# khanhptnk/psketch

Hardware: NVIDIA B200
Metric: env-steps/s (step+features+expert) (higher is better)
Workload: dtype u8

## Files before the change

### psketch_b200/csrc/psk_craft.cu

```cuda
#include <cstdio>
#include <cstdlib>
#include <cstring>
#include <atomic>
#include <mutex>

#include "psk_common.cuh"

namespace psk {

template <int W, int H, class TAB>
__device__ __forceinline__ void step_env(const TAB &st, Agent &a, uint8_t *row,
                                         const uint8_t *rd, int act, uint32_t &flags) {
    int x = a.x(), y = a.y(), dir = a.dir();
    if (act < 4) {
        dir = act;
        const int tx = x + dx_of(act), ty = y + dy_of(act);
        if (tx >= 0 && ty >= 0 && tx < W && ty < H && rd[tx * H + ty] == 0) {
            x = tx;
            y = ty;
        }
        a.set_pose(x, y, dir);
    } else if (act == PSK_ACT_USE) {
        const int fx = x + dx_of(dir), fy = y + dy_of(dir);
        if (fx >= 0 && fy >= 0 && fx < W && fy < H) {
// ... 1091 lines not shown
    const uint32_t buf_s = wbuf_s + (USE_TMA ? (uint32_t)(it & 1) * feature_tile_bytes(true, EPW, nf, 4) : 0u);
    const uint32_t trash_s = buf_s + feature_tile_bytes(USE_TMA, EPW, nf, VEC_ESZ) - 16;
    const int n16 = EPW * nf / 4;
    if (USE_TMA) {
        if (lane == 0) bulk_wait_read<1>();
        __syncwarp();
        if (KC > 0) {
#pragma unroll
            for (int i = 0; i < (n16 + 31) / 32; i++)
                if (i * 32 + lane < n16) sts_zero16(buf_s + (i * 32 + lane) * 16);
        } else {
            for (int i = lane; i < n16; i += 32) sts_zero16(buf_s + i * 16);
        }
        __syncwarp();
    }
    if (le < ne)
        scatter_features<W, H, WIN, TPE, ESZ>(buf_s + le * nf * ESZ, trash_s, cells, a, K, j);
    const uint32_t bytes = (uint32_t)ne * (uint32_t)nf * 4u;
    const bool vec_ok = (bytes & 15u) == 0 && (reinterpret_cast<uintptr_t>(gdst) & 15) == 0;
    if (USE_TMA) {
        if (vec_ok) {
            fence_async_smem();
            __syncwarp();
            if (lane == 0) bulk_store(gdst, buf_s, bytes);
        } else {
            __syncwarp();
            for (int i = lane; i < ne * nf; i += 32) {
                float t;
                asm volatile("ld.shared.f32 %0, [%1];" : "=f"(t) : "r"(buf_s + i * 4));
                gdst[i] = t;
            }
            __syncwarp();
        }
    } else if (ESZ == 4) {
        __syncwarp();
        if (vec_ok) {
            float4 *g4 = reinterpret_cast<float4 *>(gdst);
            const int m16 = (int)(bytes / 16);
            auto move16 = [&](int i) {
                float4 t;
                asm volatile("ld.shared.v4.f32 {%0,%1,%2,%3}, [%4];"
                             : "=f"(t.x), "=f"(t.y), "=f"(t.z), "=f"(t.w)
                             : "r"(buf_s + i * 16));
                sts_zero16(buf_s + i * 16);
                store_out16(g4 + i, t);
            };
            if (KC > 0 && m16 == n16) {
                constexpr int NIT = (EPW * (2 * WIN * WIN * KC + KC + 5) / 4 + 31) / 32;
#pragma unroll
                for (int i0 = 0; i0 < NIT; i0 += 4) {
                    float4 t[4];
#pragma unroll
                    for (int u = 0; u < 4; u++) {
                        const int i = (i0 + u) * 32 + lane;
                        if (i0 + u < NIT && i < n16)
                            asm volatile("ld.shared.v4.f32 {%0,%1,%2,%3}, [%4];"
                                         : "=f"(t[u].x), "=f"(t[u].y), "=f"(t[u].z), "=f"(t[u].w)
                                         : "r"(buf_s + i * 16));
                    }
#pragma unroll
                    for (int u = 0; u < 4; u++) {
                        const int i = (i0 + u) * 32 + lane;
                        if (i0 + u < NIT && i < n16) sts_zero16(buf_s + i * 16);
                    }
#pragma unroll
                    for (int u = 0; u < 4; u++) {
                        const int i = (i0 + u) * 32 + lane;
                        if (i0 + u < NIT && i < n16) store_out16(g4 + i, t[u]);
                    }
                }
            } else {
                for (int i = lane; i < m16; i += 32) move16(i);
                for (int i = m16 + lane; i < n16; i += 32) sts_zero16(buf_s + i * 16);
            }
        } else {
            for (int i = lane; i < ne * nf; i += 32) {
                float t;
                asm volatile("ld.shared.f32 %0, [%1];" : "=f"(t) : "r"(buf_s + i * 4));
                gdst[i] = t;
            }
            __syncwarp();
            for (int i = lane; i < n16; i += 32) sts_zero16(buf_s + i * 16);
        }
        __syncwarp();
    } else {
        __syncwarp();
        if (vec_ok) {
            float4 *g4 = reinterpret_cast<float4 *>(gdst);
            const int m16 = (int)(bytes / 16);
            auto move16 = [&](int i) {
                uint32_t w;
                asm volatile("ld.shared.u32 %0, [%1];" : "=r"(w) : "r"(buf_s + i * 4));
                asm volatile("st.shared.u32 [%0], %1;" ::"r"(buf_s + i * 4), "r"(0) : "memory");
                store_out16(g4 + i, widen_u8x4(w));
            };
            if (KC > 0 && m16 == n16) {
                constexpr int NIT = (EPW * (2 * WIN * WIN * KC + KC + 5) / 4 + 31) / 32;
#pragma unroll
                for (int i0 = 0; i0 < NIT; i0 += 4) {
                    uint32_t w[4];
#pragma unroll
                    for (int u = 0; u < 4; u++) {
                        const int i = (i0 + u) * 32 + lane;
                        if (i0 + u < NIT && i < n16)
                            asm volatile("ld.shared.u32 %0, [%1];" : "=r"(w[u]) : "r"(buf_s + i * 4));
                    }
#pragma unroll
                    for (int u = 0; u < 4; u++) {
                        const int i = (i0 + u) * 32 + lane;
                        if (i0 + u < NIT && i < n16)
                            asm volatile("st.shared.u32 [%0], %1;" ::"r"(buf_s + i * 4), "r"(0) : "memory");
                    }
#pragma unroll
                    for (int u = 0; u < 4; u++) {
                        const int i = (i0 + u) * 32 + lane;
                        if (i0 + u < NIT && i < n16) store_out16(g4 + i, widen_u8x4(w[u]));
                    }
                }
            } else {
                for (int i = lane; i < m16; i += 32) move16(i);
                for (int i = m16 + lane; i < n16; i += 32)
                    asm volatile("st.shared.u32 [%0], %1;" ::"r"(buf_s + i * 4), "r"(0) : "memory");
            }
        } else {
            for (int i = lane; i < ne * nf; i += 32) {
                uint32_t b;
                asm volatile("ld.shared.u8 %0, [%1];" : "=r"(b) : "r"(buf_s + i));
                gdst[i] = (float)b;
            }
            __syncwarp();
            for (int i = lane; i < n16; i += 32)
                asm volatile("st.shared.u32 [%0], %1;" ::"r"(buf_s + i * 4), "r"(0) : "memory");
        }
        __syncwarp();
    }
}

template <int W, int H, int WIN, int TPE, int KC>
__device__ __forceinline__ void warp_feature_chunk_u8(uint32_t wbuf_s, uint8_t *gdst, int ne,
                                                      const RowChunks<W, H, TPE> &cells,
                                                      const Agent &a, int K, int nf) {
    constexpr int EPW = 32 / TPE;
    if (KC > 0) {
        K = KC;
        nf = 2 * WIN * WIN * KC + KC + 5;
    }
    const int lane = threadIdx.x & 31;
    const int le = lane / TPE, j = lane % TPE;
    const uint32_t trash_s = wbuf_s + feature_tile_bytes(false, EPW, nf, 1) - 16;
    if (le < ne) scatter_features<W, H, WIN, TPE, 1>(wbuf_s + le * nf, trash_s, cells, a, K, j);
    __syncwarp();
    const int n4 = EPW * nf / 4;
    const int bytes = ne * nf;
    if ((bytes & 3) == 0 && (reinterpret_cast<uintptr_t>(gdst) & 3) == 0) {
        uint32_t *g4 = reinterpret_cast<uint32_t *>(gdst);
        for (int i = lane; i < n4; i += 32) {
            uint32_t w;
            asm volatile("ld.shared.u32 %0, [%1];" : "=r"(w) : "r"(wbuf_s + i * 4));
            asm volatile("st.shared.u32 [%0], %1;" ::"r"(wbuf_s + i * 4), "r"(0) : "memory");
            if (i < bytes / 4) __stcs(g4 + i, w);
        }
    } else {
        for (int i = lane; i < bytes; i += 32) {
            uint32_t b;
            asm volatile("ld.shared.u8 %0, [%1];" : "=r"(b) : "r"(wbuf_s + i));
            gdst[i] = (uint8_t)b;
        }
        __syncwarp();
        for (int i = lane; i < n4; i += 32)
            asm volatile("st.shared.u32 [%0], %1;" ::"r"(wbuf_s + i * 4), "r"(0) : "memory");
    }
    __syncwarp();
}

template <int W, int H, int WIN, int WPB, int TPE, int KC, bool USE_TMA, typename OUT = float>
__global__ void __launch_bounds__(WPB * 32)
craft_features_kernel(const uint8_t *__restrict__ grid, const uint8_t *__restrict__ agent,
                      OUT *__restrict__ out, int64_t n, int cell_stride, int K, int nf) {
    constexpr bool OUT_U8 = sizeof(OUT) == 1;
    static_assert(!(OUT_U8 && USE_TMA), "the u8 frame uses the vector path");
    constexpr int EPW = 32 / TPE;
    extern __shared__ __align__(128) unsigned char smem_raw[];
    const int warp = threadIdx.x >> 5, lane = threadIdx.x & 31;
    const int le = lane / TPE, j = lane % TPE;
    const uint32_t wbuf_s = smem_u32(smem_raw) + (uint32_t)warp * feature_buffer_bytes(USE_TMA, EPW, nf, PSK_ESZ_FEATURES_KERNEL);
    if (!USE_TMA) feature_buffer_init<TPE, KC, USE_TMA, PSK_ESZ_FEATURES_KERNEL>(wbuf_s, nf);
    const int64_t n_chunks = (n + EPW - 1) / EPW;
    const int64_t stride = (int64_t)gridDim.x * WPB;
    int64_t ch = (int64_t)blockIdx.x * WPB + warp;
    Agent a, a_next;
    RowChunks<W, H, TPE> cells, cells_next;
    auto fetch = [&](int64_t c, Agent &ag, RowChunks<W, H, TPE> &rc) {
        int64_t e = c * EPW + le;
        if (e >= n) e = n - 1;
        ag = load_agent_ro(agent, e);
        rc.prefetch(grid + e * cell_stride, j);
    };
    if (ch < n_chunks) fetch(ch, a, cells);
    for (int it = 0; ch < n_chunks; ch += stride, it++) {
        const bool more = ch + stride < n_chunks;
        if (more) fetch(ch + stride, a_next, cells_next);
        const int64_t e0 = ch * EPW;
        const int ne = (int)((n - e0) < EPW ? (n - e0) : EPW);
        if constexpr (OUT_U8)
            warp_feature_chunk_u8<W, H, WIN, TPE, KC>(wbuf_s, out + e0 * nf, ne, cells, a, K, nf);
        else
            warp_feature_chunk<W, H, WIN, TPE, KC, USE_TMA, PSK_ESZ_FEATURES_KERNEL>(wbuf_s, it, out + e0 * nf, ne, cells, a,
                                                                                     K, nf);
        if (more) {
            a = a_next;
            cells = cells_next;
        }
    }
    if (USE_TMA && lane == 0) bulk_wait_read<0>();
}

__global__ void __launch_bounds__(256)
craft_reset_kernel(uint8_t *__restrict__ grid, uint8_t *__restrict__ agent,
                   const uint8_t *__restrict__ scen_grid, const int32_t *__restrict__ scen_idx,
                   const uint8_t *__restrict__ init_agent, const uint8_t *__restrict__ mask,
                   int64_t n, int cell_stride) {
    const int chunks = cell_stride / 16 + 2;
    const int64_t total = n * chunks;
    for (int64_t i = blockIdx.x * (int64_t)blockDim.x + threadIdx.x; i < total;
         i += (int64_t)gridDim.x * blockDim.x) {
        const int64_t e = i / chunks;
        const int c = (int)(i % chunks);
        if (mask && !mask[e]) continue;
        if (c < cell_stride / 16) {
            const uint4 v = __ldg(reinterpret_cast<const uint4 *>(
                                      scen_grid + (int64_t)scen_idx[e] * cell_stride) + c);
            reinterpret_cast<uint4 *>(grid + e * cell_stride)[c] = v;
        } else {
            const int h = c - cell_stride / 16;
            reinterpret_cast<uint4 *>(agent + e * PSK_AGENT_BYTES)[h] =
                __ldg(reinterpret_cast<const uint4 *>(init_agent + e * PSK_AGENT_BYTES) + h);
        }
    }
}

template <int W, int H>
__device__ __forceinline__ bool advance_env(const SharedTables &st, Agent &a, uint8_t *row,
                                            const uint8_t *rd, int act, const uint8_t *scen_row,
                                            const uint8_t *init_agent_row, int cell_stride,
                                            bool &success, uint32_t &flags) {
    const int timer = a.timer() - 1;
    const bool done = (act == PSK_ACT_STOP) || timer <= 0;
    if (done) {
        const int facing = facing_kind<W, H>(a, rd);
        success = st.task_len(a.task())
                      ? node_satisfied(st.node(a.task(), 0), a, facing) == 1
                      : false;
        for (int c = 0; c < cell_stride / 16; c++)
            reinterpret_cast<uint4 *>(row)[c] = __ldg(reinterpret_cast<const uint4 *>(scen_row) + c);
        const uint4 lo = __ldg(reinterpret_cast<const uint4 *>(init_agent_row));
        const uint4 hi = __ldg(reinterpret_cast<const uint4 *>(init_agent_row) + 1);
        a.w[0] = lo.x; a.w[1] = lo.y; a.w[2] = lo.z; a.w[3] = lo.w;
        a.w[4] = hi.x; a.w[5] = hi.y; a.w[6] = hi.z; a.w[7] = hi.w;
    } else {
        success = false;
        step_env<W, H>(st, a, row, rd, act, flags);
        a.set_timer(timer);
    }
    return done;
}

__device__ __forceinline__ void add_stats(unsigned long long *stats, bool done, bool success,
                                          bool counted) {
    const unsigned full = __activemask();
    const int n_done = __popc(__ballot_sync(full, done));
    const int n_succ = __popc(__ballot_sync(full, success));
    const int n_step = __popc(__ballot_sync(full, counted));
    const int leader = __ffs(full) - 1;
    if (stats && (int)(threadIdx.x & 31) == leader) {
        if (n_done) atomicAdd(stats + 0, (unsigned long long)n_done);
        if (n_succ) atomicAdd(stats + 1, (unsigned long long)n_succ);
        if (n_step) atomicAdd(stats + 2, (unsigned long long)n_step);
    }
}

template <int W, int H>
__global__ void __launch_bounds__(256)
craft_advance_kernel(const psk_craft_tables *__restrict__ T, uint8_t *__restrict__ grid,
                     uint8_t *__restrict__ agent, const uint8_t *__restrict__ action,
                     const uint8_t *__restrict__ scen_grid, const int32_t *__restrict__ scen_idx,
                     const uint8_t *__restrict__ init_agent, uint8_t *__restrict__ done_out,
                     uint8_t *__restrict__ success_out, unsigned long long *stats,
                     int32_t *err_flags, int64_t n, int cell_stride) {
    __shared__ SharedTables st;
    stage_tables(st, T);
    uint32_t flags = 0;
    for (int64_t e = blockIdx.x * (int64_t)blockDim.x + threadIdx.x; e < n;
         e += (int64_t)gridDim.x * blockDim.x) {
        Agent a = load_agent(agent, e);
        bool success;
        const bool done = advance_env<W, H>(st, a, grid + e * cell_stride,
                                            grid + e * cell_stride, action[e],
                                            scen_grid + (int64_t)scen_idx[e] * cell_stride,
                                            init_agent + e * PSK_AGENT_BYTES, cell_stride,
                                            success, flags);
        store_agent(agent, e, a);
        if (done_out) done_out[e] = done;
        if (success_out) success_out[e] = success;
        add_stats(stats, done, success, true);
    }
    if (flags && err_flags) atomicOr(err_flags, (int)flags);
}
// ... 202 lines not shown
    const int tid = threadIdx.x;
    const bool env_warp = tid < NEW;
    const int64_t grp0 = (int64_t)blockIdx.x * (NE / PSK_CHAIN_GROUP);
    auto grp = [&](int j) { return (chain_g0 + grp0 + j) & (PSK_CHAIN_GROUPS - 1); };
    const bool chain_thread = chain && tid < NE / PSK_CHAIN_GROUP &&
                              (grp0 + tid) * PSK_CHAIN_GROUP < n;
    uint32_t flags = 0;
    if (chain) {
        if (chain_thread) s_ticket[tid] = chain_enter(chain, grp(tid));
        __syncthreads();
    }
    asm volatile("griddepcontrol.launch_dependents;");
    stage_tables(st, T);
    if (!USE_TMA && !env_warp && features_out)
        feature_buffer_init<8, KC, USE_TMA, PSK_ESZ_FUSED_KERNELS>(
            smem_u32(smem_raw) + (uint32_t)((tid - NEW) >> 5) * feature_buffer_bytes(false, 4, nf, PSK_ESZ_FUSED_KERNELS),
            nf);
    if (chain) {
        if (chain_thread && !chain_wait(chain, grp(tid), s_ticket[tid])) flags = PSK_FLAG_CHAIN_TIMEOUT;
        __syncthreads();
    } else {
        asm volatile("griddepcontrol.wait;" ::: "memory");
    }
    int it = 0;
    const int64_t n_super = (n + NE - 1) / NE;
    for (int64_t sp = blockIdx.x; sp < n_super; sp += gridDim.x) {
        const int64_t e_base = sp * NE;
        const int ne_sp = (int)((n - e_base) < NE ? (n - e_base) : NE);
        {
            const uint4 *grow = reinterpret_cast<const uint4 *>(grid + e_base * CP);
            uint4 *srow = reinterpret_cast<uint4 *>(s_rows[0]);
            for (int i = tid; i < ne_sp * (CP / 16); i += NT) srow[i] = grow[i];
            const uint4 *gag = reinterpret_cast<const uint4 *>(agent + e_base * PSK_AGENT_BYTES);
            uint4 *sag = reinterpret_cast<uint4 *>(s_agent[0]);
            for (int i = tid; i < ne_sp * 2; i += NT) sag[i] = gag[i];
        }
        __syncthreads();
        const bool live = env_warp && tid < ne_sp;
        const int slot = live ? tid : 0;
        const int64_t e = e_base + slot;
        Agent a;
        const uint8_t *scen_row = nullptr;
        int n_done = 0, n_succ = 0;
        if (env_warp) {
#pragma unroll
            for (int i = 0; i < 2; i++) {
                const uint4 v = reinterpret_cast<const uint4 *>(s_agent[0])[slot * 2 + i];
                a.w[4 * i] = v.x; a.w[4 * i + 1] = v.y; a.w[4 * i + 2] = v.z; a.w[4 * i + 3] = v.w;
            }
            scen_row = scen_grid + (int64_t)scen_idx[e] * CP;
        }
        for (int t = 0; t < ticks; t++) {
            const int cur = t & 1, nxt = cur ^ 1;
            if (env_warp) {
                const uint8_t *srow = s_rows[cur] + slot * CP;
                uint8_t *nrow = s_rows[nxt] + slot * CP;
                uint32_t words[NW4 * 4];
#pragma unroll
                for (int i = 0; i < NW4; i++) {
                    const uint4 v = reinterpret_cast<const uint4 *>(srow)[i];
                    words[4 * i] = v.x; words[4 * i + 1] = v.y; words[4 * i + 2] = v.z; words[4 * i + 3] = v.w;
                    if (live) reinterpret_cast<uint4 *>(nrow)[i] = v;
                }
                const int facing = facing_kind<W, H>(a, srow);
                int dist;
                uint32_t fl = 0;
                int act = expert_env<W, H>(st, a, a.task(), words, facing, dist, fl);
                if (live) {
                    flags |= fl;
                    const int64_t o = (int64_t)t * n + e;
                    expert_out[o] = (uint8_t)act;
                    if (action_in) act = action_in[o];
                    bool success;
                    const bool done = advance_env<W, H>(st, a, nrow, srow, act, scen_row,
                                                        init_agent + e * PSK_AGENT_BYTES, CP,
                                                        success, flags);
                    if (done_out) done_out[o] = done;
                    if (success_out) success_out[o] = success;
                    n_done += done;
                    n_succ += success;
                    uint4 *sag = reinterpret_cast<uint4 *>(s_agent[nxt]) + slot * 2;
                    sag[0] = make_uint4(a.w[0], a.w[1], a.w[2], a.w[3]);
                    sag[1] = make_uint4(a.w[4], a.w[5], a.w[6], a.w[7]);
                }
            } else if (features_out) {
                const int fw = (tid - NEW) >> 5, lane = tid & 31;
                const uint32_t wbuf_s = smem_u32(smem_raw) +
                                        (uint32_t)fw * feature_buffer_bytes(USE_TMA, EPW, nf, PSK_ESZ_FUSED_KERNELS);
                OUT *fout = features_out + (int64_t)(t % feat_ring) * n * nf;
                for (int c = 0; c < SPW / EPW; c++) {
                    const int s0 = fw * SPW + c * EPW;
                    if (s0 >= ne_sp) break;
                    const int ne = (ne_sp - s0) < EPW ? (ne_sp - s0) : EPW;
                    int se = s0 + lane / TPE;
                    if (se >= ne_sp) se = s0;
                    Agent b;
#pragma unroll
                    for (int i = 0; i < 2; i++) {
                        const uint4 v = reinterpret_cast<const uint4 *>(s_agent[cur])[se * 2 + i];
                        b.w[4 * i] = v.x; b.w[4 * i + 1] = v.y; b.w[4 * i + 2] = v.z; b.w[4 * i + 3] = v.w;
                    }
                    RowChunks<W, H, TPE> cells;
                    cells.load(s_rows[cur] + se * CP, lane % TPE);
                    if constexpr (sizeof(OUT) == 1) {
                        static_assert(sizeof(OUT) != 1 || (!USE_TMA && PSK_ESZ_FUSED_KERNELS == 1), "u8 frame: vector path, u8 tile");
                        warp_feature_chunk_u8<W, H, WIN, TPE, KC>(wbuf_s, fout + (e_base + s0) * nf, ne, cells,
                                                                  b, K, nf);
                    } else {
                        warp_feature_chunk<W, H, WIN, TPE, KC, USE_TMA, PSK_ESZ_FUSED_KERNELS>(
                            wbuf_s, it, fout + (e_base + s0) * nf, ne, cells, b, K, nf);
                    }
                    it++;
                }
            }
            __syncthreads();
        }
        if (env_warp) {
            if (live) {
                store_agent(agent, e, a);
                const uint8_t *frow = s_rows[ticks & 1] + slot * CP;
#pragma unroll
                for (int i = 0; i < NW4; i++)
                    reinterpret_cast<uint4 *>(grid + e * CP)[i] = reinterpret_cast<const uint4 *>(frow)[i];
            }
            const int d = __reduce_add_sync(0xffffffffu, n_done);
            const int sc = __reduce_add_sync(0xffffffffu, n_succ);
            const int lv = __reduce_add_sync(0xffffffffu, live ? ticks : 0);
            if (stats && (tid & 31) == 0) {
                if (d) atomicAdd(stats + 0, (unsigned long long)d);
                if (sc) atomicAdd(stats + 1, (unsigned long long)sc);
                if (lv) atomicAdd(stats + 2, (unsigned long long)lv);
            }
        }
        __syncthreads();
    }
    if (chain_thread) chain_leave(chain, grp(tid), s_ticket[tid]);
    if (USE_TMA && !env_warp && (tid & 31) == 0) bulk_wait_read<0>();
    if (flags && err_flags) atomicOr(err_flags, (int)flags);
}

static int num_sms() {
    static int sms[PSK_MAX_DEVICES] = {0};
    const int dev = current_device();
    if (!sms[dev]) {
        int n = 0;
        cudaDeviceGetAttribute(&n, cudaDevAttrMultiProcessorCount, dev);
        sms[dev] = n > 0 ? n : 148;
    }
    return sms[dev];
}

enum TuneKey { TUNE_ROLLOUT_VARIANT, TUNE_ROLLOUT_TMA, TUNE_TICK_VARIANT, TUNE_TICK_TMA,
               TUNE_TICK_PERSIST, TUNE_FEAT_PERSIST, TUNE_TICK_PDL, TUNE_STEP_VARIANT,
               TUNE_TILE_CHAIN, TUNE_COUNT };
static const char *const tune_names[TUNE_COUNT] = {
    "rollout_variant", "rollout_tma", "tick_variant", "tick_tma", "tick_persist", "feat_persist",
    "tick_pdl", "step_variant", "tile_chain"};
static std::atomic<int> tune_val[TUNE_COUNT];
static std::once_flag tune_once;
static void tune_init() {
    for (int i = 0; i < TUNE_COUNT; i++) {
        char name[64] = "PSK_";
        size_t j = 4;
        for (const char *c = tune_names[i]; *c && j + 1 < sizeof(name); c++)
            name[j++] = (char)(*c >= 'a' && *c <= 'z' ? *c - 32 : *c);
        name[j] = 0;
        const char *v = getenv(name);
        tune_val[i].store(v ? atoi(v) : -1);
    }
}
static inline int tune(TuneKey k) {
    std::call_once(tune_once, tune_init);
    return tune_val[k].load(std::memory_order_relaxed);
}

static inline int grid_for(int64_t n, int block, int ctas_per_sm) {
    int64_t need = (n + block - 1) / block;
    int64_t cap = (int64_t)num_sms() * ctas_per_sm;
    return (int)(need < cap ? (need > 0 ? need : 1) : cap);
}

static inline int check(cudaError_t e) { return e == cudaSuccess ? PSK_OK : PSK_ERR_CUDA; }

static const psk_craft_tables *device_tables(const psk_craft_tables *caller_tables, cudaStream_t st) {
    constexpr int MAX_DEV = PSK_MAX_DEVICES, SLOTS = 8;
    struct Slot {
        psk_craft_tables host;
        psk_craft_tables *dev = nullptr;
    };
    struct PerDevice {
        Slot slot[SLOTS];
        int used = 0, last = 0, next_victim = 0;
    };
    static PerDevice cache[MAX_DEV];
    static std::mutex mu;
    int dev = 0;
    if (cudaGetDevice(&dev) != cudaSuccess || dev < 0 || dev >= MAX_DEV) return nullptr;
    psk_craft_tables canon = *caller_tables;
    memset(canon.ws_recipes, 0, sizeof(canon.ws_recipes));
    for (int r = 0; r < canon.n_recipes && r < PSK_MAX_RECIPES; r++)
        canon.ws_recipes[canon.recipes[r][1] & (PSK_MAX_KINDS - 1)] |= (uint16_t)(1u << r);
    const psk_craft_tables *t = &canon;
    std::lock_guard<std::mutex> lock(mu);
    PerDevice &c = cache[dev];
    if (c.used && memcmp(&c.slot[c.last].host, t, sizeof(psk_craft_tables)) == 0) return c.slot[c.last].dev;
    for (int i = 0; i < c.used; ++i)
        if (memcmp(&c.slot[i].host, t, sizeof(psk_craft_tables)) == 0) {
            c.last = i;
            return c.slot[i].dev;
        }
    int i;
    if (c.used < SLOTS) {
        i = c.used;
        if (cudaMalloc(&c.slot[i].dev, sizeof(psk_craft_tables)) != cudaSuccess) return nullptr;
        ++c.used;
    } else {
        i = c.next_victim;
        c.next_victim = (c.next_victim + 1) % SLOTS;
        if (cudaDeviceSynchronize() != cudaSuccess) return nullptr;
    }
    memset(&c.slot[i].host, 0xFF, sizeof(psk_craft_tables));
    if (cudaMemcpyAsync(c.slot[i].dev, t, sizeof(psk_craft_tables), cudaMemcpyHostToDevice, st) != cudaSuccess)
        return nullptr;
    if (cudaStreamSynchronize(st) != cudaSuccess) return nullptr;
    c.slot[i].host = *t;
    c.last = i;
    return c.slot[i].dev;
}
static uint32_t *chain_counters(const psk_craft_state &s, int64_t *g0) {
    static uint32_t *ctr[PSK_MAX_DEVICES] = {nullptr};
    static std::mutex mu;
    const int64_t n = s.n;
    if (tune(TUNE_TILE_CHAIN) == 0 || tune(TUNE_TICK_PDL) == 0) return nullptr;
    if ((n + PSK_CHAIN_GROUP - 1) / PSK_CHAIN_GROUP > PSK_CHAIN_GROUPS) return nullptr;
    constexpr uintptr_t GROUP_BYTES = (uintptr_t)PSK_CHAIN_GROUP * PSK_AGENT_BYTES;
    if (reinterpret_cast<uintptr_t>(s.agent) % GROUP_BYTES) return nullptr;
    *g0 = (int64_t)(reinterpret_cast<uintptr_t>(s.agent) / GROUP_BYTES);
    const int dev = current_device();
    std::lock_guard<std::mutex> lock(mu);
    if (!ctr[dev]) {
        const size_t bytes = (size_t)2 * PSK_CHAIN_GROUPS * sizeof(uint32_t);
        if (cudaMalloc(&ctr[dev], bytes) != cudaSuccess) return nullptr;
        if (cudaMemset(ctr[dev], 0, bytes) != cudaSuccess || cudaDeviceSynchronize() != cudaSuccess) {
            cudaFree(ctr[dev]);
            ctr[dev] = nullptr;
        }
    }
    return ctr[dev];
}

#define PSK_DT(var)                                   \
    const psk_craft_tables *var = device_tables(t, st); \
    if (!var) return PSK_ERR_CUDA

template <int W, int H, int WIN> struct Config {
    static constexpr int CP = ((W * H + 63) / 64) * 64;
    static constexpr int TPE = 8;
    static constexpr bool BITBOARD = W * H <= 128;

    static bool matches(const psk_craft_tables *t) {
        return t->width == W && t->height == H && t->window_w == WIN && t->window_h == WIN &&
               t->n_kinds <= PSK_MAX_INV;
    }
    static int nf(const psk_craft_tables *t) { return 2 * WIN * WIN * t->n_kinds + t->n_kinds + 5; }

    static int step(const psk_craft_tables *t, psk_craft_state s, const uint8_t *action,
                    const uint8_t *active, float *reward, int32_t *err, cudaStream_t st) {
        PSK_DT(dt);
        int mode = tune(TUNE_STEP_VARIANT);
        if (mode < 0 || mode > 2) mode = 0;
        if (mode == 2 && CP != 64) mode = 1;
        cudaLaunchConfig_t cfg = {};
        cfg.blockDim = dim3(mode == 0 ? 256 : 64);
        cfg.gridDim = dim3((unsigned)(mode == 0 ? grid_for(s.n, 256, 8) : grid_for(s.n, 64, 32)));
        cfg.stream = st;
        cudaLaunchAttribute attr[1];
        attr[0].id = cudaLaunchAttributeProgrammaticStreamSerialization;
        attr[0].val.programmaticStreamSerializationAllowed = 1;
        cfg.attrs = attr;
        cfg.numAttrs = tune(TUNE_TICK_PDL) != 0 ? 1 : 0;
        const int cell_stride = s.cell_stride;
        const int64_t n = s.n;
        if (mode == 0)
            return check(cudaLaunchKernelEx(&cfg, craft_step_kernel<W, H, 0>, dt, s.grid, s.agent, action,
                                            active, reward, err, n, cell_stride));
        if constexpr (CP == 64) {
            if (mode == 2)
                return check(cudaLaunchKernelEx(&cfg, craft_step_kernel<W, H, 2>, dt, s.grid, s.agent,
                                                action, active, reward, err, n, cell_stride));
        }
        return check(cudaLaunchKernelEx(&cfg, craft_step_kernel<W, H, 1>, dt, s.grid, s.agent, action,
                                        active, reward, err, n, cell_stride));
    }
    static int satisfies(const psk_craft_tables *t, psk_craft_state s, const uint8_t *task,
                         uint8_t *out, cudaStream_t st) {
        PSK_DT(dt);
        craft_satisfies_kernel<W, H><<<grid_for(s.n, 256, 8), 256, 0, st>>>(
            dt, s.grid, s.agent, task, out, s.n, s.cell_stride);
        return check(cudaGetLastError());
    }
    static int expert(const psk_craft_tables *t, psk_craft_state s, const uint8_t *task,
                      uint8_t *action, int16_t *dist, int32_t *err, cudaStream_t st) {
        PSK_DT(dt);
        if constexpr (BITBOARD)
            craft_expert_kernel<W, H><<<grid_for(s.n, 128, 8), 128, 0, st>>>(
                dt, s.grid, s.agent, task, action, dist, err, s.n, s.cell_stride);
        else if constexpr (W <= 16 && H <= 32)
            craft_expert_half_rows_kernel<W, H><<<grid_for((s.n + 1) / 2, 4, 16), 128, 0, st>>>(
                dt, s.grid, s.agent, task, action, dist, err, s.n, s.cell_stride);
        else
            craft_expert_rows_kernel<W, H><<<grid_for(s.n, 4, 16), 128, 0, st>>>(
                dt, s.grid, s.agent, task, action, dist, err, s.n, s.cell_stride);
        return check(cudaGetLastError());
    }
    static int find_closest(const psk_craft_tables *t, psk_craft_state s, const uint8_t *kind,
                            uint8_t *goal, int16_t *len, uint8_t *seq, int seq_cap,
                            cudaStream_t st) {
        PSK_DT(dt);
        if constexpr (BITBOARD)
            craft_find_closest_kernel<W, H><<<grid_for(s.n, 128, 8), 128, 0, st>>>(
                dt, s.grid, s.agent, kind, goal, len, seq, seq_cap, s.n, s.cell_stride);
        else
            craft_find_closest_rows_kernel<W, H><<<grid_for(s.n, 4, 16), 128, 0, st>>>(
                s.grid, s.agent, kind, goal, len, seq, seq_cap, s.n, s.cell_stride);
        return check(cudaGetLastError());
    }
    template <bool TMA, typename OUT = float>
    static int features_impl(const psk_craft_tables *t, psk_craft_state s, OUT *out,
                             cudaStream_t st) {
        constexpr int WPB = 4, EPW = 32 / TPE;
        const int f = nf(t);
        const size_t smem = (size_t)WPB * feature_buffer_bytes(TMA, EPW, f, PSK_ESZ_FEATURES_KERNEL);
        auto kern = t->n_kinds == 21 ? craft_features_kernel<W, H, WIN, WPB, TPE, 21, TMA, OUT>
                                     : craft_features_kernel<W, H, WIN, WPB, TPE, 0, TMA, OUT>;
        static size_t configured_on[PSK_MAX_DEVICES] = {0};
        size_t &configured = configured_on[current_device()];
        if (configured != smem) {
            if (cudaFuncSetAttribute(craft_features_kernel<W, H, WIN, WPB, TPE, 21, TMA, OUT>,
                                     cudaFuncAttributeMaxDynamicSharedMemorySize, (int)smem) != cudaSuccess ||
                cudaFuncSetAttribute(craft_features_kernel<W, H, WIN, WPB, TPE, 0, TMA, OUT>,
                                     cudaFuncAttributeMaxDynamicSharedMemorySize, (int)smem) != cudaSuccess)
                return PSK_ERR_CUDA;
            configured = smem;
        }
        int per_sm = (int)((224 * 1024) / (smem + 1024));
        if (per_sm > 16) per_sm = 16;
        const int64_t ctas = (s.n + (int64_t)WPB * EPW - 1) / ((int64_t)WPB * EPW);
        int64_t g = (int64_t)num_sms() * (per_sm > 0 ? per_sm : 1);
        const int persist = tune(TUNE_FEAT_PERSIST) > 0;
        if (g > ctas || !persist) g = ctas > 0 ? ctas : 1;
        kern<<<(int)g, WPB * 32, smem, st>>>(s.grid, s.agent, out, s.n, s.cell_stride, t->n_kinds, f);
        return check(cudaGetLastError());
    }
    static int features(const psk_craft_tables *t, psk_craft_state s, float *out, int impl,
                        cudaStream_t st) {
        if ((reinterpret_cast<uintptr_t>(out) & 15) != 0) impl = 1;
        return impl == 2 ? features_impl<true>(t, s, out, st) : features_impl<false>(t, s, out, st);
    }
    static int features_u8(const psk_craft_tables *t, psk_craft_state s, uint8_t *out, cudaStream_t st) {
        return features_impl<false, uint8_t>(t, s, out, st);
    }
    static int advance(const psk_craft_tables *t, psk_craft_state s, psk_craft_episodes ep,
                       const uint8_t *action, uint8_t *done, uint8_t *success,
                       unsigned long long *stats, int32_t *err, cudaStream_t st) {
        PSK_DT(dt);
        craft_advance_kernel<W, H><<<grid_for(s.n, 256, 8), 256, 0, st>>>(
            dt, s.grid, s.agent, action, ep.scen_grid, ep.scen_idx, ep.init_agent, done, success,
            stats, err, s.n, s.cell_stride);
        return check(cudaGetLastError());
    }
    template <int NE, int NFW, bool TMA, typename OUT = float>
    static int tick_variant(const psk_craft_tables *t, psk_craft_state s, psk_craft_episodes ep,
                            const uint8_t *action_in, OUT *features_out, uint8_t *expert_out,
                            uint8_t *done, uint8_t *success, unsigned long long *stats,
                            int32_t *err, cudaStream_t st, int adv_first) {
        constexpr int EPW = 32 / TPE;
        const int f = nf(t);
        const size_t smem = (size_t)NFW * feature_buffer_bytes(TMA, EPW, f, PSK_ESZ_FUSED_KERNELS);
        auto kern = t->n_kinds == 21 ? craft_tick_kernel<W, H, WIN, NE, NFW, 21, TMA, OUT>
                                     : craft_tick_kernel<W, H, WIN, NE, NFW, 0, TMA, OUT>;
        static size_t configured_on[PSK_MAX_DEVICES] = {0};
        size_t &configured = configured_on[current_device()];
        if (configured != smem) {
            if (cudaFuncSetAttribute(craft_tick_kernel<W, H, WIN, NE, NFW, 21, TMA, OUT>,
                                     cudaFuncAttributeMaxDynamicSharedMemorySize, (int)smem) != cudaSuccess ||
                cudaFuncSetAttribute(craft_tick_kernel<W, H, WIN, NE, NFW, 0, TMA, OUT>,
                                     cudaFuncAttributeMaxDynamicSharedMemorySize, (int)smem) != cudaSuccess)
                return PSK_ERR_CUDA;
            configured = smem;
        }
        const size_t static_smem = sizeof(SharedTables) + (size_t)NE * (CP + 32);
        int per_sm = (int)((224 * 1024) / (smem + static_smem + 1024));
        const int by_threads = 2048 / (NE + NFW * 32);
        if (per_sm > by_threads) per_sm = by_threads;
        const int64_t tiles = (s.n + NE - 1) / NE;
        int64_t g = (int64_t)num_sms() * (per_sm > 0 ? per_sm : 1);
        const int persist = tune(TUNE_TICK_PERSIST) > 0;
        if (g > tiles || !persist) g = tiles > 0 ? tiles : 1;
        PSK_DT(dt);
        const int pdl = tune(TUNE_TICK_PDL) != 0;
        cudaLaunchConfig_t cfg = {};
        cfg.gridDim = dim3((unsigned)g);
        cfg.blockDim = dim3(NE + NFW * 32);
        cfg.dynamicSmemBytes = smem;
        cfg.stream = st;
        cudaLaunchAttribute attr[1];
        attr[0].id = cudaLaunchAttributeProgrammaticStreamSerialization;
        attr[0].val.programmaticStreamSerializationAllowed = 1;
        cfg.attrs = attr;
        cfg.numAttrs = pdl ? 1 : 0;
        const int cell_stride = s.cell_stride, K = t->n_kinds;
        int64_t chain_g0 = 0;
        uint32_t *chain = (g == tiles && pdl && !TMA) ? chain_counters(s, &chain_g0) : nullptr;
        return check(cudaLaunchKernelEx(&cfg, kern, dt, s.grid, s.agent, action_in, ep.scen_grid,
                                        ep.scen_idx, ep.init_agent, features_out, expert_out, done,
                                        success, stats, err, s.n, cell_stride, K, f, adv_first, chain,
                                        chain_g0));
    }
    template <int NE, int NFW, bool TMA, typename OUT = float>
    static int rollout_variant(const psk_craft_tables *t, psk_craft_state s, psk_craft_episodes ep,
                               int ticks, const uint8_t *action_in, OUT *features_out,
                               int feat_ring, uint8_t *expert_out, uint8_t *done,
                               uint8_t *success, unsigned long long *stats, int32_t *err,
                               cudaStream_t st) {
        constexpr int EPW = 32 / TPE;
        const int f = nf(t);
        const size_t smem = (size_t)NFW * feature_buffer_bytes(TMA, EPW, f, PSK_ESZ_FUSED_KERNELS);
        auto kern = t->n_kinds == 21 ? craft_rollout_kernel<W, H, WIN, NE, NFW, 21, TMA, OUT>
                                     : craft_rollout_kernel<W, H, WIN, NE, NFW, 0, TMA, OUT>;
        static size_t configured_on[PSK_MAX_DEVICES] = {0};
        size_t &configured = configured_on[current_device()];
        if (configured != smem) {
            if (cudaFuncSetAttribute(craft_rollout_kernel<W, H, WIN, NE, NFW, 21, TMA, OUT>,
                                     cudaFuncAttributeMaxDynamicSharedMemorySize, (int)smem) != cudaSuccess ||
                cudaFuncSetAttribute(craft_rollout_kernel<W, H, WIN, NE, NFW, 0, TMA, OUT>,
                                     cudaFuncAttributeMaxDynamicSharedMemorySize, (int)smem) != cudaSuccess)
                return PSK_ERR_CUDA;
            configured = smem;
        }
        const int64_t tiles = (s.n + NE - 1) / NE;
        PSK_DT(dt);
        cudaLaunchConfig_t cfg = {};
        cfg.gridDim = dim3((unsigned)(tiles > 0 ? tiles : 1));
        cfg.blockDim = dim3(rollout_threads(NE, NFW));
        cfg.dynamicSmemBytes = smem;
        cfg.stream = st;
        cudaLaunchAttribute attr[1];
        attr[0].id = cudaLaunchAttributeProgrammaticStreamSerialization;
        attr[0].val.programmaticStreamSerializationAllowed = 1;
        cfg.attrs = attr;
        cfg.numAttrs = 1;
        const int cell_stride = s.cell_stride, K = t->n_kinds;
        int64_t chain_g0 = 0;
        uint32_t *chain = chain_counters(s, &chain_g0);
        return check(cudaLaunchKernelEx(&cfg, kern, dt, s.grid, s.agent, action_in, ep.scen_grid,
                                        ep.scen_idx, ep.init_agent, features_out, feat_ring,
                                        expert_out, done, success, stats, err, s.n, cell_stride, K,
                                        f, ticks, chain, chain_g0));
    }
    static int rollout(const psk_craft_tables *t, psk_craft_state s, psk_craft_episodes ep, int ticks,
                       const uint8_t *action_in, float *features_out, int feat_ring,
                       uint8_t *expert_out, uint8_t *done, uint8_t *success,
                       unsigned long long *stats, int32_t *err, cudaStream_t st) {
        if constexpr (!BITBOARD) {
            return PSK_ERR_UNSUPPORTED;
        } else if constexpr (WIN != 3) {
            return PSK_ERR_UNSUPPORTED;
        } else {
            const int env_tma = tune(TUNE_ROLLOUT_TMA), env_variant = tune(TUNE_ROLLOUT_VARIANT);
            const int tma = env_tma >= 0 ? env_tma : (s.n > 196608 ? 1 : 0);
            const int variant = env_variant >= 0 ? env_variant : 2;
#define PSK_ROLLOUT_ARGS t, s, ep, ticks, action_in, features_out, feat_ring, expert_out, done, success, stats, err, st
            if (variant == 2)
                return tma ? rollout_variant<32, 2, true>(PSK_ROLLOUT_ARGS)
                           : rollout_variant<32, 2, false>(PSK_ROLLOUT_ARGS);
            if (variant == 3)
                return tma ? rollout_variant<16, 2, true>(PSK_ROLLOUT_ARGS)
                           : rollout_variant<16, 2, false>(PSK_ROLLOUT_ARGS);
            if (variant == 4)
                return tma ? rollout_variant<16, 1, true>(PSK_ROLLOUT_ARGS)
                           : rollout_variant<16, 1, false>(PSK_ROLLOUT_ARGS);
            return tma ? rollout_variant<64, 2, true>(PSK_ROLLOUT_ARGS)
                       : rollout_variant<64, 2, false>(PSK_ROLLOUT_ARGS);
#undef PSK_ROLLOUT_ARGS
        }
    }
    static int tick_u8(const psk_craft_tables *t, psk_craft_state s, psk_craft_episodes ep,
                       const uint8_t *action_in, uint8_t *features_out, uint8_t *expert_out, uint8_t *done,
                       uint8_t *success, unsigned long long *stats, int32_t *err, cudaStream_t st,
                       int adv_first) {
        if constexpr (!BITBOARD) {
            return PSK_ERR_UNSUPPORTED;
        } else if constexpr (WIN != 3) {
            return tick_variant<64, 2, false, uint8_t>(t, s, ep, action_in, features_out, expert_out, done,
                                                       success, stats, err, st, adv_first);
        } else {
            return tick_variant<32, 2, false, uint8_t>(t, s, ep, action_in, features_out, expert_out, done,
                                                       success, stats, err, st, adv_first);
        }
    }
    static int rollout_u8(const psk_craft_tables *t, psk_craft_state s, psk_craft_episodes ep, int ticks,
                          const uint8_t *action_in, uint8_t *features_out, int feat_ring,
                          uint8_t *expert_out, uint8_t *done, uint8_t *success,
                          unsigned long long *stats, int32_t *err, cudaStream_t st) {
        if constexpr (!BITBOARD || WIN != 3) {
            return PSK_ERR_UNSUPPORTED;
        } else {
            return rollout_variant<32, 2, false, uint8_t>(t, s, ep, ticks, action_in, features_out, feat_ring,
                                                          expert_out, done, success, stats, err, st);
        }
    }
    static int tick_fused(const psk_craft_tables *t, psk_craft_state s, psk_craft_episodes ep,
                          const uint8_t *action_in, float *features_out, uint8_t *expert_out,
                          uint8_t *done, uint8_t *success, unsigned long long *stats,
                          int32_t *err, cudaStream_t st, int adv_first) {
        if constexpr (!BITBOARD) {
            return PSK_ERR_UNSUPPORTED;
        } else {
        const int env_variant = tune(TUNE_TICK_VARIANT), env_tma = tune(TUNE_TICK_TMA);
        const bool big = s.n > 262144;
        const int variant = env_variant >= 0 ? env_variant : 4;
        const int tma = env_tma >= 0 ? env_tma : (big ? 1 : 0);
#define PSK_TV(NE, NFW)                                                                          \
    return tma ? tick_variant<NE, NFW, true>(t, s, ep, action_in, features_out, expert_out, done, \
                                             success, stats, err, st, adv_first)                 \
               : tick_variant<NE, NFW, false>(t, s, ep, action_in, features_out, expert_out, done, \
                                              success, stats, err, st, adv_first)
        if constexpr (WIN != 3) {
            (void)variant;
            PSK_TV(64, 2);
        } else {
            switch (variant) {
                case 1: PSK_TV(128, 4);
                case 2: PSK_TV(32, 1);
                case 3: PSK_TV(64, 4);
                case 4: PSK_TV(32, 2);
                default: PSK_TV(64, 2);
            }
        }
#undef PSK_TV
        }
    }
};

using Medium = Config<8, 8, 3>;
using Large = Config<10, 10, 5>;
using Stress16 = Config<16, 16, 3>;
using Stress32 = Config<32, 32, 3>;
using Stress64 = Config<64, 64, 3>;

#define PSK_DISPATCH(t, CALL)                             \
    do {                                                  \
        if (Medium::matches(t)) return Medium::CALL;      \
        if (Large::matches(t)) return Large::CALL;        \
        if (Stress16::matches(t)) return Stress16::CALL;  \
        if (Stress32::matches(t)) return Stress32::CALL;  \
        if (Stress64::matches(t)) return Stress64::CALL;  \
        return PSK_ERR_UNSUPPORTED;                       \
    } while (0)

static bool state_ok(const psk_craft_tables *t, const psk_craft_state &s) {
    if (!t || s.n < 0) return false;
    if (s.n == 0) return true;
    if (!s.grid || !s.agent) return false;
    const int need = ((t->width * t->height + 63) / 64) * 64;
    if (s.cell_stride != need) return false;
    if ((reinterpret_cast<uintptr_t>(s.grid) & 15) || (reinterpret_cast<uintptr_t>(s.agent) & 31))
        return false;
    return true;
}

}

using namespace psk;

extern "C" {

const char *psk_version(void) { return "psketch_b200 0.2 sm_100a"; }

int psk_set_tuning(const char *key, int32_t value) {
    if (!key) return PSK_ERR_BADARG;
    tune(TUNE_ROLLOUT_VARIANT);
    for (int i = 0; i < TUNE_COUNT; i++)
        if (strcmp(key, tune_names[i]) == 0) {
            tune_val[i].store(value);
            return PSK_OK;
        }
    return PSK_ERR_BADARG;
}

int psk_get_tuning(const char *key, int32_t *value) {
    if (!key || !value) return PSK_ERR_BADARG;
    for (int i = 0; i < TUNE_COUNT; i++)
        if (strcmp(key, tune_names[i]) == 0) {
            *value = tune((TuneKey)i);
            return PSK_OK;
        }
    return PSK_ERR_BADARG;
}

int psk_craft_supported(const psk_craft_tables *t) {
    if (!t) return 0;
    return Medium::matches(t) || Large::matches(t) || Stress16::matches(t) || Stress32::matches(t) ||
           Stress64::matches(t);
}

int psk_craft_n_features(const psk_craft_tables *t) {
    if (!psk_craft_supported(t)) return -1;
    return 2 * t->window_w * t->window_h * t->n_kinds + t->n_kinds + 5;
}

int psk_craft_step(const psk_craft_tables *t, psk_craft_state s, const uint8_t *action,
                   const uint8_t *active, float *reward, int32_t *err_flags, void *stream) {
    if (!state_ok(t, s) || (!action && s.n)) return PSK_ERR_BADARG;
    if (s.n == 0) return PSK_OK;
    PSK_DISPATCH(t, step(t, s, action, active, reward, err_flags, (cudaStream_t)stream));
}

int psk_craft_features(const psk_craft_tables *t, psk_craft_state s, float *out, int impl,
                       void *stream) {
    if (!state_ok(t, s) || (!out && s.n)) return PSK_ERR_BADARG;
    if (s.n == 0) return PSK_OK;
    PSK_DISPATCH(t, features(t, s, out, impl, (cudaStream_t)stream));
}

int psk_craft_features_u8(const psk_craft_tables *t, psk_craft_state s, uint8_t *out, void *stream) {
    if (!state_ok(t, s) || (!out && s.n)) return PSK_ERR_BADARG;
    if (s.n == 0) return PSK_OK;
    PSK_DISPATCH(t, features_u8(t, s, out, (cudaStream_t)stream));
}

int psk_craft_satisfies(const psk_craft_tables *t, psk_craft_state s, const uint8_t *task,
                        uint8_t *out, void *stream) {
    if (!state_ok(t, s) || (!out && s.n)) return PSK_ERR_BADARG;
    if (s.n == 0) return PSK_OK;
    PSK_DISPATCH(t, satisfies(t, s, task, out, (cudaStream_t)stream));
}

int psk_craft_expert(const psk_craft_tables *t, psk_craft_state s, const uint8_t *task,
                     uint8_t *action, int16_t *dist, int32_t *err_flags, void *stream) {
    if (!state_ok(t, s) || (!action && s.n)) return PSK_ERR_BADARG;
    if (s.n == 0) return PSK_OK;
    PSK_DISPATCH(t, expert(t, s, task, action, dist, err_flags, (cudaStream_t)stream));
}

int psk_craft_find_closest(const psk_craft_tables *t, psk_craft_state s, const uint8_t *kind,
                           uint8_t *goal, int16_t *length, uint8_t *seq, int32_t seq_cap,
                           void *stream) {
    if (!state_ok(t, s) || ((!kind || !goal || !length) && s.n) || seq_cap < 0)
        return PSK_ERR_BADARG;
    if (s.n == 0) return PSK_OK;
    PSK_DISPATCH(t, find_closest(t, s, kind, goal, length, seq, seq_cap, (cudaStream_t)stream));
}

int psk_craft_reset(psk_craft_state s, psk_craft_episodes ep, const uint8_t *mask, void *stream) {
    if (s.n < 0 || s.cell_stride <= 0 || s.cell_stride % 64) return PSK_ERR_BADARG;
    if (s.n == 0) return PSK_OK;
    if (!s.grid || !s.agent || !ep.scen_grid || !ep.scen_idx || !ep.init_agent)
        return PSK_ERR_BADARG;
    const int64_t total = s.n * (s.cell_stride / 16 + 2);
    craft_reset_kernel<<<grid_for(total, 256, 8), 256, 0, (cudaStream_t)stream>>>(
        s.grid, s.agent, ep.scen_grid, ep.scen_idx, ep.init_agent, mask, s.n, s.cell_stride);
    return check(cudaGetLastError());
// ... 137 lines not shown
```

Measured before the change: 4.197 billion.

## Widen u8 feature stores to 16B, max shared carveout, retune u8 kernel shapes

Adds a 16-byte vectorized path for copying u8 feature tiles from shared memory to global, unrolled when the kind count is a compile-time constant, with a byte-wise tail for non-multiple sizes. For u8 kernels it also requests the maximum shared-memory carveout. It changes the default u8 tick and rollout launch shape from 32 envs × 2 feature warps to 32 × 1, with new env knobs to pick among shapes, and adds a Python probe script to time and hash the variants. The aim is fewer store instructions and better occupancy for the u8 output path, at the cost of some byte-store tail handling and possibly less feature-warp parallelism.

Result: no change. 4.197 billion, median of 6 (+0.0%).

```diff
diff --git a/profiles/u8_split_probe.py b/profiles/u8_split_probe.py
--- /dev/null
+++ b/profiles/u8_split_probe.py
@@ -0,0 +1,148 @@
+#!/usr/bin/env python
+import argparse
+import hashlib
+import json
+import os
+import subprocess
+import sys
+
+import numpy as np
+import torch
+
+ROOT = os.path.dirname(os.path.dirname(os.path.abspath(__file__)))
+sys.path.insert(0, ROOT)
+from bench import load_workload, time_kernel
+from psketch_b200 import _lib
+from psketch_b200.tables import CraftTables
+from psketch_b200.vec import VecCraft
+
+U8_SHAPES = {0: "32+2", 1: "32+1", 2: "64+1"}
+
+
+def gpu_info():
+    try:
+        q = subprocess.run(["nvidia-smi", "--query-gpu=name,power.limit,clocks.max.sm", "--format=csv,noheader"],
+                           capture_output=True, text=True, timeout=30).stdout.strip()
+    except Exception as ex:
+        q = repr(ex)
+    return {"nvidia_smi": q, "torch_name": torch.cuda.get_device_name(0)}
+
+
+def has_u8_knobs():
+    try:
+        _lib.set_tuning(rollout_u8_variant=-1, tick_u8_variant=-1)
+        return True
+    except _lib.PskError:
+        return False
+
+
+def digest(n, tables, wl):
+    knobs = has_u8_knobs()
+    shapes = sorted(U8_SHAPES) if knobs else [None] * len(U8_SHAPES)
+    h = hashlib.sha256()
+    env = VecCraft.from_instances(tables, wl["grids"], wl["env"], wl["pos"], wl["task"], max_timesteps=40)
+    g = torch.Generator(device="cpu").manual_seed(7)
+    T = 8
+    ring = torch.empty((T + 1, n, tables.n_features), dtype=torch.uint8, device=env.device)
+    frame = torch.empty((n, tables.n_features), dtype=torch.uint8, device=env.device)
+    for rnd in range(2):
+        for s in shapes:
+            if s is not None:
+                _lib.set_tuning(rollout_u8_variant=s, tick_u8_variant=s)
+            acts = None
+            if rnd == 1:
+                acts = torch.multinomial(torch.tensor([.19, .19, .19, .19, .2, .04]), T * n, replacement=True,
+                                         generator=g).to(torch.uint8).view(T, n).to(env.device)
+            ring.fill_(0xAB)
+            out = env.rollout(T, actions=acts, features_out=ring)
+            for k in ("expert", "done", "success"):
+                h.update(out[k].cpu().numpy().tobytes())
+            h.update(ring.cpu().numpy().tobytes())
+            for adv in (False, True):
+                a1 = torch.randint(0, 6, (n,), generator=g, dtype=torch.uint8).to(env.device)
+                o = env.tick(actions=a1, features_out=frame, advance_first=adv)
+                for k in ("expert", "done", "success"):
+                    h.update(o[k].cpu().numpy().tobytes())
+                h.update(frame.cpu().numpy().tobytes())
+    env.check_errors()
+    h.update(env.grid.cpu().numpy().tobytes())
+    h.update(env.agent.cpu().numpy().tobytes())
+    h.update(env.stats.cpu().numpy().tobytes())
+    if knobs:
+        _lib.set_tuning(rollout_u8_variant=-1, tick_u8_variant=-1)
+    return h.hexdigest()
+
+
+def main():
+    ap = argparse.ArgumentParser()
+    ap.add_argument("--n", type=int, default=65536)
+    ap.add_argument("--ticks", type=int, default=8)
+    ap.add_argument("--rounds", type=int, default=5)
+    ap.add_argument("--tag", default="default")
+    ap.add_argument("--out", default=None)
+    args = ap.parse_args()
+    n, T = args.n, args.ticks
+    tables = CraftTables()
+    nf = tables.n_features
+    wl = load_workload(n)
+    env = VecCraft.from_instances(tables, wl["grids"], wl["env"], wl["pos"], wl["task"], max_timesteps=40)
+    dev = env.device
+    knobs = has_u8_knobs()
+    u8_ring = torch.empty((2 * T, n, nf), dtype=torch.uint8, device=dev)
+    f32_ring = torch.empty((2 * T, n, nf), dtype=torch.float32, device=dev)
+    cnt = [0]
+    r_out, t_out = {}, {}
+
+    def half(ring):
+        s = (cnt[0] % 2) * T
+        cnt[0] += 1
+        return ring[s:s + T]
+
+    def frame():
+        cnt[0] += 1
+        return u8_ring[cnt[0] % (2 * T)]
+
+    def knob(key, s, fn):
+        def f():
+            if s is not None:
+                _lib.set_tuning(**{key: s})
+            fn()
+        return f
+
+    cases = {
+        "env_only": (lambda: env.rollout(T, features_out=None, out=r_out), T),
+        "f32_rollout": (lambda: env.rollout(T, features_out=half(f32_ring), out=r_out), T),
+        "features_u8": (lambda: env.features_u8(out=frame()), 1),
+    }
+    for s in (sorted(U8_SHAPES) if knobs else [None]):
+        name = "v%d" % s if s is not None else "default"
+        cases["u8_rollout_" + name] = (
+            knob("rollout_u8_variant", s, lambda: env.rollout(T, features_out=half(u8_ring), out=r_out)), T)
+        cases["u8_tick_" + name] = (knob("tick_u8_variant", s, lambda: env.tick(features_out=frame(), out=t_out)), 1)
+    snap = env.snapshot()
+    times = {k: [] for k in cases}
+    for rnd in range(args.rounds):
+        for k, (fn, per_launch) in cases.items():
+            env.restore(snap)
+            dt = time_kernel(fn, torch, inner=2 * T // per_launch if per_launch > 1 else 2 * T, reps=20)
+            times[k].append(dt * 1e6 / per_launch)
+    if knobs:
+        _lib.set_tuning(rollout_u8_variant=-1, tick_u8_variant=-1)
+    env.restore(snap)
+    env.check_errors()
+    res = {"n": n, "ticks_per_launch": T, "rounds": args.rounds, "gpu": gpu_info(), "tag": args.tag,
+           "lib": os.environ.get("PSK_LIB") or "in-tree",
+           "us_per_tick_median": {k: float(np.median(v)) for k, v in times.items()},
+           "us_per_tick_all": times,
+           "u8_shapes": U8_SHAPES if knobs else "library without rollout_u8_variant / tick_u8_variant (32 + 2)",
+           "bytes_per_env_step": {"u8_frame": nf, "f32_frame": 4 * nf},
+           "outputs_sha256": digest(n, tables, wl)}
+    path = args.out or os.path.join(ROOT, "profiles", "bench_runs", "u8_split_probe_%s.json" % args.tag)
+    os.makedirs(os.path.dirname(path), exist_ok=True)
+    with open(path, "w") as f:
+        json.dump(res, f, indent=1)
+    print(json.dumps({"tag": args.tag, "median": res["us_per_tick_median"], "sha256": res["outputs_sha256"]}))
+
+
+if __name__ == "__main__":
+    main()
diff --git a/psketch_b200/csrc/psk_craft.cu b/psketch_b200/csrc/psk_craft.cu
--- a/psketch_b200/csrc/psk_craft.cu
+++ b/psketch_b200/csrc/psk_craft.cu
@@ -1267,7 +1267,46 @@
     __syncwarp();
     const int n4 = EPW * nf / 4;
     const int bytes = ne * nf;
-    if ((bytes & 3) == 0 && (reinterpret_cast<uintptr_t>(gdst) & 3) == 0) {
+    if ((reinterpret_cast<uintptr_t>(gdst) & 15) == 0) {
+        const int n16 = (EPW * nf + 15) / 16, m16 = bytes / 16, r = bytes - 16 * m16;
+        uint4 *g16 = reinterpret_cast<uint4 *>(gdst);
+        auto out16 = [&](int i, const uint4 &v) {
+            if (i < m16) {
+                __stcs(g16 + i, v);
+            } else if (i == m16 && r) {
+                for (int b = 0; b < r; b++) {
+                    const uint32_t w = b < 4 ? v.x : (b < 8 ? v.y : (b < 12 ? v.z : v.w));
+                    gdst[16 * i + b] = (uint8_t)(w >> (8 * (b & 3)));
+                }
+            }
+        };
+        if (KC > 0) {
+            constexpr int NIT = (EPW * (2 * WIN * WIN * KC + KC + 5) + 16 * 32 - 1) / (16 * 32);
+            uint4 v[NIT];
+#pragma unroll
+            for (int u = 0; u < NIT; u++) {
+                const int i = u * 32 + lane;
+                if (i < n16)
+                    asm volatile("ld.shared.v4.u32 {%0,%1,%2,%3}, [%4];"
+                                 : "=r"(v[u].x), "=r"(v[u].y), "=r"(v[u].z), "=r"(v[u].w)
+                                 : "r"(wbuf_s + i * 16));
+            }
+#pragma unroll
+            for (int u = 0; u < NIT; u++)
+                if (u * 32 + lane < n16) sts_zero16(wbuf_s + (u * 32 + lane) * 16);
+#pragma unroll
+            for (int u = 0; u < NIT; u++) out16(u * 32 + lane, v[u]);
+        } else {
+            for (int i = lane; i < n16; i += 32) {
+                uint4 v;
+                asm volatile("ld.shared.v4.u32 {%0,%1,%2,%3}, [%4];"
+                             : "=r"(v.x), "=r"(v.y), "=r"(v.z), "=r"(v.w)
+                             : "r"(wbuf_s + i * 16));
+                sts_zero16(wbuf_s + i * 16);
+                out16(i, v);
+            }
+        }
+    } else if ((bytes & 3) == 0 && (reinterpret_cast<uintptr_t>(gdst) & 3) == 0) {
         uint32_t *g4 = reinterpret_cast<uint32_t *>(gdst);
         for (int i = lane; i < n4; i += 32) {
             uint32_t w;
@@ -1776,10 +1815,10 @@
 
 enum TuneKey { TUNE_ROLLOUT_VARIANT, TUNE_ROLLOUT_TMA, TUNE_TICK_VARIANT, TUNE_TICK_TMA,
                TUNE_TICK_PERSIST, TUNE_FEAT_PERSIST, TUNE_TICK_PDL, TUNE_STEP_VARIANT,
-               TUNE_TILE_CHAIN, TUNE_COUNT };
+               TUNE_TILE_CHAIN, TUNE_ROLLOUT_U8_VARIANT, TUNE_TICK_U8_VARIANT, TUNE_COUNT };
 static const char *const tune_names[TUNE_COUNT] = {
     "rollout_variant", "rollout_tma", "tick_variant", "tick_tma", "tick_persist", "feat_persist",
-    "tick_pdl", "step_variant", "tile_chain"};
+    "tick_pdl", "step_variant", "tile_chain", "rollout_u8_variant", "tick_u8_variant"};
 static std::atomic<int> tune_val[TUNE_COUNT];
 static std::once_flag tune_once;
 static void tune_init() {
@@ -1873,6 +1912,15 @@
     return ctr[dev];
 }
 
+template <typename KERN> static int set_smem_attributes(KERN kern, size_t smem, bool max_carveout) {
+    if (cudaFuncSetAttribute(kern, cudaFuncAttributeMaxDynamicSharedMemorySize, (int)smem) != cudaSuccess)
+        return 1;
+    if (max_carveout && cudaFuncSetAttribute(kern, cudaFuncAttributePreferredSharedMemoryCarveout,
+                                             (int)cudaSharedmemCarveoutMaxShared) != cudaSuccess)
+        return 1;
+    return 0;
+}
+
 #define PSK_DT(var)                                   \
     const psk_craft_tables *var = device_tables(t, st); \
     if (!var) return PSK_ERR_CUDA
@@ -2006,10 +2054,8 @@
         static size_t configured_on[PSK_MAX_DEVICES] = {0};
         size_t &configured = configured_on[current_device()];
         if (configured != smem) {
-            if (cudaFuncSetAttribute(craft_tick_kernel<W, H, WIN, NE, NFW, 21, TMA, OUT>,
-                                     cudaFuncAttributeMaxDynamicSharedMemorySize, (int)smem) != cudaSuccess ||
-                cudaFuncSetAttribute(craft_tick_kernel<W, H, WIN, NE, NFW, 0, TMA, OUT>,
-                                     cudaFuncAttributeMaxDynamicSharedMemorySize, (int)smem) != cudaSuccess)
+            if (set_smem_attributes(craft_tick_kernel<W, H, WIN, NE, NFW, 21, TMA, OUT>, smem, sizeof(OUT) == 1) ||
+                set_smem_attributes(craft_tick_kernel<W, H, WIN, NE, NFW, 0, TMA, OUT>, smem, sizeof(OUT) == 1))
                 return PSK_ERR_CUDA;
             configured = smem;
         }
@@ -2055,10 +2101,8 @@
         static size_t configured_on[PSK_MAX_DEVICES] = {0};
         size_t &configured = configured_on[current_device()];
         if (configured != smem) {
-            if (cudaFuncSetAttribute(craft_rollout_kernel<W, H, WIN, NE, NFW, 21, TMA, OUT>,
-                                     cudaFuncAttributeMaxDynamicSharedMemorySize, (int)smem) != cudaSuccess ||
-                cudaFuncSetAttribute(craft_rollout_kernel<W, H, WIN, NE, NFW, 0, TMA, OUT>,
-                                     cudaFuncAttributeMaxDynamicSharedMemorySize, (int)smem) != cudaSuccess)
+            if (set_smem_attributes(craft_rollout_kernel<W, H, WIN, NE, NFW, 21, TMA, OUT>, smem, sizeof(OUT) == 1) ||
+                set_smem_attributes(craft_rollout_kernel<W, H, WIN, NE, NFW, 0, TMA, OUT>, smem, sizeof(OUT) == 1))
                 return PSK_ERR_CUDA;
             configured = smem;
         }
@@ -2109,30 +2153,43 @@
 #undef PSK_ROLLOUT_ARGS
         }
     }
+    static int u8_shape(int knob) { return knob >= 0 && knob <= 2 ? knob : 1; }
     static int tick_u8(const psk_craft_tables *t, psk_craft_state s, psk_craft_episodes ep,
                        const uint8_t *action_in, uint8_t *features_out, uint8_t *expert_out, uint8_t *done,
                        uint8_t *success, unsigned long long *stats, int32_t *err, cudaStream_t st,
                        int adv_first) {
+#define PSK_TV8(NE, NFW) \
+    return tick_variant<NE, NFW, false, uint8_t>(t, s, ep, action_in, features_out, expert_out, done, success, stats, err, st, adv_first)
         if constexpr (!BITBOARD) {
             return PSK_ERR_UNSUPPORTED;
         } else if constexpr (WIN != 3) {
-            return tick_variant<64, 2, false, uint8_t>(t, s, ep, action_in, features_out, expert_out, done,
-                                                       success, stats, err, st, adv_first);
+            PSK_TV8(64, 2);
         } else {
-            return tick_variant<32, 2, false, uint8_t>(t, s, ep, action_in, features_out, expert_out, done,
-                                                       success, stats, err, st, adv_first);
-        }
+            switch (u8_shape(tune(TUNE_TICK_U8_VARIANT))) {
+                case 0: PSK_TV8(32, 2);
+                case 2: PSK_TV8(64, 1);
+                default: PSK_TV8(32, 1);
+            }
+        }
+#undef PSK_TV8
     }
     static int rollout_u8(const psk_craft_tables *t, psk_craft_state s, psk_craft_episodes ep, int ticks,
                           const uint8_t *action_in, uint8_t *features_out, int feat_ring,
                           uint8_t *expert_out, uint8_t *done, uint8_t *success,
                           unsigned long long *stats, int32_t *err, cudaStream_t st) {
+#define PSK_RV8(NE, NFW)                                                                                   \
+    return rollout_variant<NE, NFW, false, uint8_t>(t, s, ep, ticks, action_in, features_out, feat_ring, \
+                                                    expert_out, done, success, stats, err, st)
         if constexpr (!BITBOARD || WIN != 3) {
             return PSK_ERR_UNSUPPORTED;
         } else {
-            return rollout_variant<32, 2, false, uint8_t>(t, s, ep, ticks, action_in, features_out, feat_ring,
-                                                          expert_out, done, success, stats, err, st);
-        }
+            switch (u8_shape(tune(TUNE_ROLLOUT_U8_VARIANT))) {
+                case 0: PSK_RV8(32, 2);
+                case 2: PSK_RV8(64, 1);
+                default: PSK_RV8(32, 1);
+            }
+        }
+#undef PSK_RV8
     }
     static int tick_fused(const psk_craft_tables *t, psk_craft_state s, psk_craft_episodes ep,
                           const uint8_t *action_in, float *features_out, uint8_t *expert_out,
```
